# dome272/Paella

Measured on AMD Instinct MI355X. Metric: images/sec (whole node) + single-image ms, 256x256 @ 8 steps, higher is better.
Workload: dtype f32; 1 GPU; BASELINE configs[1]: Paella 573M-class (stand-in blocks=[4,8,4]) (570.3M params), 32x32 tokens = 256 px, 8 steps, CFG 8.0, CLIP-H-text only (S=4), batch 1 per GPU, + VQGAN f8 decode; denoiser=570m, sample_steps=8, noise=philox, submission=hip-graph replay, world_size_observed=1

## Files before the change

paella_amd/csrc/gemm.hip:

```cpp
#include "common.h"
#include "gemm_device.h"
#include "philox.h"
#include <stdio.h>
#include <stdlib.h>
#include "test_hooks.h"
#include <atomic>
#include <mutex>
#include <string>
#include <type_traits>
#include <utility>
#include <vector>

typedef unsigned int u32x4 __attribute__((ext_vector_type(4)));
typedef __bf16 bf16x8 __attribute__((ext_vector_type(8)));

template <typename F, int... Is>
__device__ __forceinline__ void static_for_impl(F& f, std::integer_sequence<int, Is...>) { (f(std::integral_constant<int, Is>{}), ...); }
template <int N, typename F>
__device__ __forceinline__ void static_for(F& f) { static_for_impl(f, std::make_integer_sequence<int, N>{}); }

struct SkPlan {
    int tiles_m, tiles_n;
    int KT;
    unsigned U;
    unsigned G;
    FastDiv dKT, dTM, dQ, dQ1;
    unsigned q, r;
    int stagger;
    int gm;
};

template <bool GROUPED>
__device__ __forceinline__ void sk_tile_coords(const SkPlan& p, int tile, int& tile_m, int& tile_n) {
    if (!GROUPED || p.gm >= p.tiles_m) {
        tile_n = (int)fast_div((unsigned)tile, p.dTM);
        tile_m = tile - tile_n * p.tiles_m;
    } else {
        const int width = p.gm * p.tiles_n;
        const int grp = tile / width, rem = tile - grp * width;
        const int first_m = grp * p.gm;
        const int gsz = min(p.tiles_m - first_m, p.gm);
        tile_n = rem / gsz;
        tile_m = first_m + (rem - tile_n * gsz);
    }
}

__device__ __forceinline__ unsigned sk_start(const SkPlan& p, unsigned g) { return g * p.q + min(g, p.r); }
__device__ __forceinline__ unsigned sk_owner(const SkPlan& p, unsigned x) {
    const unsigned big = p.r * (p.q + 1);
    return x < big ? fast_div(x, p.dQ1) : p.r + fast_div(x - big, p.dQ);
}

template <int AUX = 0>
__device__ __forceinline__ void dma_b128_to_lds(__amdgpu_buffer_rsrc_t rsrc, float* lds_wave_base, unsigned voffset, int soffset) {
#if defined(__HIP_DEVICE_COMPILE__)
    __builtin_amdgcn_raw_ptr_buffer_load_lds(rsrc, (__attribute__((address_space(3))) void*)lds_wave_base, 16, voffset, soffset, 0, AUX);
#endif
}
#ifndef PAELLA_RING_W_AUX
#define PAELLA_RING_W_AUX 2
#endif

__device__ __forceinline__ f32x4 mma_bf16(const f32x4 w, const f32x4 a, const f32x4 c) {
    return __builtin_amdgcn_mfma_f32_16x16x32_bf16(__builtin_bit_cast(bf16x8, w), __builtin_bit_cast(bf16x8, a), c, 0, 0, 0);
}

#ifdef PAELLA_GEMM_CLOCK_PROBE
__device__ unsigned long long g_clock_probe[2];
extern "C" int paella_probe_gemm_clock(unsigned long long* out2) {
    HIP_CHECK_RET(hipDeviceSynchronize());
    HIP_CHECK_RET(hipMemcpyFromSymbol(out2, HIP_SYMBOL(g_clock_probe), 2 * sizeof(unsigned long long)));
    return PAELLA_OK;
}
#endif

struct TileRes {
    int BM, BN;
    int tile_floats;
    int stage_floats;
    int flag_off;
    int tail_floats;
    int grn_scr;
    int lds_bytes;
    int side_samples;
};
constexpr TileRes tile_res(int WM, int WN, int TM, int TN, int APRO, bool TAIL, int BK, int RING) {
    const int BM = WM * TM * 16, BN = WN * TN * 16;
    const bool big = RING > 0 && WM * WN == 8;
    const int aux = RING == 0 ? 0 : (big && APRO == 1) ? 576 : APRO == 1 ? 512 : APRO == 4 ? 320 : 0;
    const int tile = (BM + BN) * BK, stage = tile + aux;
    const int flag_off = RING > 0 ? RING * stage : 2 * stage;
    const int tail = TAIL ? BM * WN * 2 : 0;
    const int scr = (RING > 0 && !big) ? WM * WN * TN * 16 : 0;
    return TileRes{BM, BN, tile, stage, flag_off, tail, scr, (flag_off + 16 + tail + scr) * 4, big ? 16 : 8};
}
constexpr int tile_wg_per_cu(int WM, int WN, int TM, int TN, int PD, int APRO, bool TAIL, int BK, bool DMA, int RING, bool BF) {
    const int NW = WM * WN, blocks = TM * TN;
    if (RING > 0) {
        const int wish = NW == 8 ? 1 : blocks == 1 ? (RING == 3 ? 5 : 4) : (blocks == 2 ? ((BF && APRO == 2 && TM == 2) ? 3 : 4) : 3);
        const int fit = (160 * 1024) / tile_res(WM, WN, TM, TN, APRO, TAIL, BK, RING).lds_bytes;
        return fit < wish ? (fit < 1 ? 1 : fit) : wish;
    }
    if (TAIL && DMA) return 4;
    if (TAIL && NW == 8 && blocks == 4) return 4;
    if (WM == 2 && WN == 2 && blocks == 1 && PD == 2 && BK == 32 && (APRO == 0 || APRO == 3)) return 5;
    if (DMA && NW == 4 && blocks == 16) return 2;
    if (NW == 8 && WM * TM == 8 && WN * TN == 4 && PD == 2 && BK == 32 && APRO == 0 && !TAIL) return 4;
    return 1;
}

template <int WM, int WN, int TM, int TN, int PD, int APRO, bool TAIL = false, int BK = 32, bool DMA = false, int RING = 0, bool BF = false, int EPI = EPI_RUNTIME, bool REQ = false>
__global__ __launch_bounds__(64 * WM * WN, tile_wg_per_cu(WM, WN, TM, TN, PD, APRO, TAIL, BK, DMA, RING, BF)) void gemm_nt_kernel(GemmArgs g, SkPlan p, float* __restrict__ slabs,
                                                               unsigned* __restrict__ tickets, unsigned slab_bytes) {
    constexpr TileRes RES = tile_res(WM, WN, TM, TN, APRO, TAIL, BK, RING);
    constexpr int BM = RES.BM, BN = RES.BN;
    constexpr int SL = BK / 4;
    constexpr int KG = BK / 16;
    constexpr int NW = WM * WN, NT = 64 * NW;
    constexpr int RP = NT / SL;
    constexpr int LA = (BM * SL + NT - 1) / NT, LB = (BN * SL + NT - 1) / NT;
    static_assert(NW == 4 || NW == 8, "4 or 8 waves per workgroup");
    static_assert(!REQ || TAIL, "the request form exists for the fused tail only");
    static_assert(PD == 1 || PD == 2, "prefetch ring depth 1 or 2");
    static_assert(BK == 32 || BK == 64, "K step of 32 or 64");
    static_assert(!BF || ((DMA || RING > 0) && (APRO == 0 || APRO == 2) && BK == 32), "bf16 operands: direct-to-LDS / ring variants, no operand transform");
    constexpr int ESZ = BF ? 2 : 4;
    constexpr bool DMA_W = DMA || RING > 0, DMA_A = (DMA && (APRO == 0 || APRO == 2)) || RING > 0;
    static_assert(!DMA || (PD == 1 && BK == 32 && (BM * SL) % NT == 0 && (BN * SL) % NT == 0), "DMA variant: 1-deep, K step 32, whole passes");
    constexpr bool PP = RING == 2;
    static_assert(!PP || (BF && NW == 8 && WM == 2 && WN == 4 && TM == 8 && TN == 4 && (APRO == 0 || APRO == 2)), "ping-pong tile: bf16 operands, 2 x 4 waves of 128x64 wave tiles");
    static_assert(RING == 0 || (RING >= 2 && RING <= 4 && !DMA && PD == 1 && BK == 32 && !TAIL && APRO != 3 && (NW == 4 || (TM == 4 && TN == 4 && RING == 3) || PP) && (BM * SL) % NT == 0 && (BN * SL) % NT == 0),
                  "ring variant: 3 or 4 LDS stages (2 for the ping-pong tile), 4 waves (or 8 waves of 64x64 / 128x64 wave tiles), K step 32, whole passes, no implicit convolution");
    static_assert(APRO != 4 || RING > 0, "the GRN-from-raw-statistics prologue exists on ring tiles only");
    constexpr bool BIG = RING > 0 && NW == 8;
    static_assert(!BIG || APRO != 4, "the 8-wave ring tile has no GRN-from-raw-statistics prologue");
    constexpr bool GRN_SIDE = RING > 0 && (APRO == 1 || APRO == 4);
    constexpr bool GRN_FIN = RING > 0 && !BIG;
    constexpr int TILE_FLOATS = RES.tile_floats, STAGE_FLOATS = RES.stage_floats, FLAG_OFF = RES.flag_off, TAIL_FLOATS = RES.tail_floats;
    static_assert(RES.side_samples == (BIG ? 16 : 8) && (RES.grn_scr > 0) == GRN_FIN, "tile_res() and the kernel agree on which ring tiles are BIG");
    __shared__ __attribute__((aligned(16))) float smem[RES.lds_bytes / 4];

    const unsigned G = p.G;
    unsigned gid = blockIdx.x;
    {
        const unsigned q = G >> 3, r = G & 7;
        const unsigned xcd = gid & 7, idx = gid >> 3;
        gid = xcd * q + min(xcd, r) + idx;
    }
    const unsigned u0 = sk_start(p, gid);
    const int n = (int)(p.q + (gid < p.r ? 1u : 0u));
    __builtin_assume(n > 0);
#ifdef PAELLA_GEMM_CLOCK_PROBE
    const unsigned long long cp_t0 = __builtin_readcyclecounter(), cp_w0 = wall_clock64();
#endif
    const int KT = p.KT;

    const int tid = threadIdx.x;
    const int lane_k = tid & 63;
    const int lane = lane_k;
    const int wave = __builtin_amdgcn_readfirstlane(tid >> 6);
    const int wm = wave / WN, wn = wave % WN;
    const int r16 = lane & 15, kq = lane >> 4;
    const int ldrow = tid / SL, ldc4 = tid % SL;

    f32x4 acc[TM][TN];
#pragma unroll
    for (int i = 0; i < TM; ++i)
#pragma unroll
        for (int j = 0; j < TN; ++j) acc[i][j] = f32x4{0.f, 0.f, 0.f, 0.f};

    struct Stage {
        f32x4 a[LA];
        f32x4 s[APRO == 1 ? LA : 1];
        f32x4 t;
        f32x4 b[LB];
        bool kok;
        bool ok[APRO == 3 ? LA : 1];
    };
    Stage R[PD];

    int ltile = (int)fast_div(u0, p.dKT);
    int lkt = (int)(u0 - (unsigned)ltile * (unsigned)KT);
    auto rsrc_of = [](const void* ptr, size_t bytes) {
        return __builtin_amdgcn_make_buffer_rsrc(const_cast<void*>(ptr), 0, (int)(bytes > 0xffffffffull ? 0xffffffffull : bytes), 0x00020000);
    };
    const char* const Abase = BF ? reinterpret_cast<const char*>(g.A16) : reinterpret_cast<const char*>(g.A);
    const char* const Wbase = BF ? reinterpret_cast<const char*>(g.W16) : reinterpret_cast<const char*>(g.W);
    const size_t a_bytes = APRO == 3 ? (size_t)(g.M / (g.cv.Ho * g.cv.Wo)) * g.cv.Hi * g.cv.Wi * g.cv.C * sizeof(float)
                                     : ((size_t)(g.M - 1) * g.lda + g.K) * ESZ;
    const size_t w_bytes = ((size_t)(g.N - 1) * g.ldw + g.K) * ESZ;
    __amdgpu_buffer_rsrc_t rsrcA = rsrc_of(Abase, a_bytes), rsrcW = rsrc_of(Wbase, w_bytes);
    __amdgpu_buffer_rsrc_t rsrcS = rsrc_of(g.A, 16);
    const __amdgpu_buffer_rsrc_t rsrcT = rsrc_of((APRO == 1 || APRO == 4) ? g.a_shift : g.A, (APRO == 1 || APRO == 4) ? (size_t)g.K * sizeof(float) : 16);
    const __amdgpu_buffer_rsrc_t rsrcG = rsrc_of(APRO == 4 ? g.grn_gamma : g.A, APRO == 4 ? (size_t)g.K * sizeof(float) : 16);
    unsigned aoff[LA], soff[APRO == 1 ? LA : 1], boff[LB];
    unsigned aux_s_off2 = 0;
    unsigned aux_s_off = 0;
    int cy[APRO == 3 ? LA : 1], cx[APRO == 3 ? LA : 1];
    int ltap = 0, lc0 = 0;
    auto set_tile = [&](int tile) __attribute__((always_inline)) {
        int tile_m, tile_n;
        sk_tile_coords<(BM >= 64)>(p, tile, tile_m, tile_n);
        const int m0 = tile_m * BM, n0 = tile_n * BN;
        size_t a_base;
        int img0 = 0, smp0 = 0;
        if (APRO == 3) {
            img0 = m0 / (g.cv.Ho * g.cv.Wo);
            a_base = (size_t)img0 * g.cv.Hi * g.cv.Wi * g.cv.C * sizeof(float);
        } else {
            a_base = (size_t)m0 * g.lda * ESZ;
        }
        rsrcA = rsrc_of(Abase + a_base, a_bytes - a_base);
        const size_t w_base = (size_t)n0 * g.ldw * ESZ;
        rsrcW = rsrc_of(Wbase + w_base, w_bytes - w_base);
        if (APRO == 1 || APRO == 4) {
            smp0 = (int)fast_div((unsigned)m0, g.a_rps_div);
            const size_t s_bytes = (size_t)(fast_div((unsigned)(g.M - 1), g.a_rps_div) + 1) * g.K * sizeof(float), s_base = (size_t)smp0 * g.K * sizeof(float);
            rsrcS = rsrc_of((APRO == 4 ? g.grn_gx : g.a_scale) + (size_t)smp0 * g.K, s_bytes - s_base);
        }
#pragma unroll
        for (int i = 0; i < LA; ++i) {
            const int gmc = min(m0 + ldrow + i * RP, g.M - 1);
            if (APRO == 3) {
                const int hw = g.cv.Ho * g.cv.Wo;
                const int bimg = gmc / hw, rem = gmc - bimg * hw;
                const int yo = rem / g.cv.Wo, xo = rem - yo * g.cv.Wo;
                cy[i] = yo * g.cv.stride;
                cx[i] = xo * g.cv.stride;
                aoff[i] = (unsigned)(bimg - img0) * (unsigned)(g.cv.Hi * g.cv.Wi);
            } else {
                aoff[i] = (unsigned)(gmc - m0) * (unsigned)g.lda * (unsigned)ESZ + (unsigned)((DMA_A ? (ldc4 ^ (ldrow & (SL - 1))) : ldc4) * 16);
            }
            if (APRO == 1 && RING == 0) soff[i] = ((unsigned)((int)fast_div((unsigned)gmc, g.a_rps_div) - smp0) * (unsigned)g.K + (unsigned)(ldc4 * 4)) * 4u;
        }
        if (GRN_SIDE) {
            const int last = (int)fast_div((unsigned)(g.M - 1), g.a_rps_div) - smp0;
            aux_s_off = ((unsigned)min(lane_k >> 3, last) * (unsigned)g.K + (unsigned)((lane_k & 7) * 4)) * 4u;
            if (BIG) aux_s_off2 = ((unsigned)min(8 + (lane_k >> 3), last) * (unsigned)g.K + (unsigned)((lane_k & 7) * 4)) * 4u;
        }
#pragma unroll
        for (int i = 0; i < LB; ++i) boff[i] = (unsigned)(min(n0 + ldrow + i * RP, g.N - 1) - n0) * (unsigned)g.ldw * (unsigned)ESZ + (unsigned)((DMA_W ? (ldc4 ^ (ldrow & (SL - 1))) : ldc4) * 16);
    };
    set_tile(ltile);
    if (APRO == 3) {
        ltap = (lkt * BK) / g.cv.C;
        lc0 = lkt * BK - ltap * g.cv.C;
    }
    float fr_mu[APRO == 2 ? TM : 1], fr_rs[APRO == 2 ? TM : 1];
    float fr_mu_lo[APRO == 2 ? TM : 1];
    bool ln_dir[APRO == 2 ? TM : 1];
    constexpr bool BF_FIX = BF && APRO == 2 && NW == 4;
    bool ln_any = false;
    int ln_row0 = 0;
    const int ln_tile0 = ltile;
    auto ln_row_stats = [&]() __attribute__((always_inline)) {
        if constexpr (APRO == 2) {
            int ln_tm, ln_tn;
            sk_tile_coords<(BM >= 64)>(p, ln_tile0, ln_tm, ln_tn);
            ln_row0 = ln_tm * BM;
            int lane_l = (NW == 8 && BF) ? (int)__builtin_amdgcn_mbcnt_hi(~0u, __builtin_amdgcn_mbcnt_lo(~0u, 0u)) : lane_k;
            asm volatile("" : "+v"(lane_l));
            const int r16 = lane_l & 15;
            if (PP || g.ln_row) {
#pragma unroll
                for (int i = 0; i < TM; ++i) {
                    const int gmc = min(ln_tm * BM + (wm * TM + i) * 16 + r16, g.M - 1);
                    const f32x4 v = *reinterpret_cast<const f32x4*>(g.ln_row + (size_t)gmc * 4);
                    fr_mu[i] = v[0]; fr_rs[i] = v[1]; fr_mu_lo[i] = v[2];
                    if constexpr (BF) {
                        ln_dir[i] = false;
                        const bool pre = g.A != nullptr && v[3] > g.ln_fold_ratio;
                        if (pre) { fr_mu[i] = 0.f; fr_rs[i] = 1.f; }
                        if (g.ln_guard_count) ln_any = ln_any || __builtin_amdgcn_ballot_w64(pre) != 0;
                    } else {
                        ln_dir[i] = __builtin_amdgcn_ballot_w64(v[3] > g.ln_fold_ratio) != 0;
                        ln_any = ln_any || ln_dir[i];
                    }
                }
                if (g.ln_guard_count && ln_any && lane_l == 0) atomicAdd(g.ln_guard_count, 1u);
                return;
            }
            const int nch = g.ln_nblk >> 1;
#pragma unroll
            for (int i = 0; i < TM; ++i) {
                const int gmc = min(ln_tm * BM + (wm * TM + i) * 16 + r16, g.M - 1);
                const float* st0 = g.ln_stats + (size_t)gmc * g.ln_nblk * 2;
                const bool vec = (((size_t)gmc * g.ln_nblk) & 1) == 0;
                RowStatAcc acc;
                if (vec) {
                    const f32x4* stp = reinterpret_cast<const f32x4*>(st0);
                    int j = kq;
                    for (; j + 12 < nch; j += 16) {
                        const f32x4 v0 = stp[j], v1 = stp[j + 4], v2 = stp[j + 8], v3 = stp[j + 12];
                        acc.add(v0[0], v0[1]); acc.add(v0[2], v0[3]); acc.add(v1[0], v1[1]); acc.add(v1[2], v1[3]);
                        acc.add(v2[0], v2[1]); acc.add(v2[2], v2[3]); acc.add(v3[0], v3[1]); acc.add(v3[2], v3[3]);
                    }
                    for (; j < nch; j += 4) {
                        const f32x4 v0 = stp[j];
                        acc.add(v0[0], v0[1]); acc.add(v0[2], v0[3]);
                    }
                    if ((g.ln_nblk & 1) && kq == 0) acc.add(st0[2 * (g.ln_nblk - 1)], st0[2 * (g.ln_nblk - 1) + 1]);
                } else {
                    for (int j = kq; j < g.ln_nblk; j += 4) acc.add(st0[2 * j], st0[2 * j + 1]);
                }
                acc.S += __shfl_xor(acc.S, 16, 64); acc.Q += __shfl_xor(acc.Q, 16, 64); acc.M += __shfl_xor(acc.M, 16, 64);
                acc.S += __shfl_xor(acc.S, 32, 64); acc.Q += __shfl_xor(acc.Q, 32, 64); acc.M += __shfl_xor(acc.M, 32, 64);
                acc.finish(g.K, g.ln_eps, fr_mu[i], fr_rs[i]);
                fr_mu_lo[i] = (float)(acc.S / (double)g.K - (double)fr_mu[i]);
                ln_dir[i] = (!BF || (BF_FIX && g.A != nullptr)) && __builtin_amdgcn_ballot_w64(fabsf(fr_mu[i]) * fr_rs[i] > g.ln_fold_ratio) != 0;
                ln_any = ln_any || ln_dir[i];
            }
            if (g.ln_guard_count && ln_any && lane_k == 0) atomicAdd(g.ln_guard_count, 1u);
        }
    };
    auto ln_fix = [&](f32x4& a, int i, int kbase) __attribute__((always_inline)) {
        if constexpr (APRO == 2 && !BF) {
            if (ln_dir[i]) {
#pragma unroll
                for (int e = 0; e < 4; ++e) a[e] = (kbase + e < g.K) ? ((a[e] - fr_mu[i]) - fr_mu_lo[i]) * fr_rs[i] : 0.f;
            }
        }
        if constexpr (BF_FIX) {
            if (ln_dir[i]) {
                const int gm = min(ln_row0 + (wm * TM + i) * 16 + r16, g.M - 1);
                const float* src = g.A + (size_t)gm * g.lda + 2 * kbase;
                typedef __bf16 bf16x4_t __attribute__((ext_vector_type(4)));
                f32x4 v = *reinterpret_cast<const f32x4*>(src);
#pragma unroll
                for (int e = 0; e < 4; ++e) v[e] = ((v[e] - fr_mu[i]) - fr_mu_lo[i]) * fr_rs[i];
                const bf16x4_t lo = __builtin_convertvector(v, bf16x4_t);
                v = *reinterpret_cast<const f32x4*>(src + 4);
#pragma unroll
                for (int e = 0; e < 4; ++e) v[e] = ((v[e] - fr_mu[i]) - fr_mu_lo[i]) * fr_rs[i];
                const bf16x4_t hi = __builtin_convertvector(v, bf16x4_t);
                a = __builtin_bit_cast(f32x4, __builtin_shufflevector(lo, hi, 0, 1, 2, 3, 4, 5, 6, 7));
            }
        }
    };
    int kt_cur = 0;

    auto load_unit = [&](Stage& r, int dma_slot) __attribute__((always_inline)) {
        float* dAs = smem + dma_slot * (RING > 0 ? STAGE_FLOATS : TILE_FLOATS) + (wave * (64 / SL)) * BK;
        float* dBs = dAs + BM * BK;
        const int kofs = lkt * (BK * 4);
        if constexpr (RING > 0) {
#pragma unroll
            for (int i = 0; i < LA; ++i) dma_b128_to_lds(rsrcA, dAs + i * RP * BK, aoff[i], kofs);
#pragma unroll
            for (int i = 0; i < LB; ++i) dma_b128_to_lds<((BIG || TM * TN != 1) ? 0 : PAELLA_RING_W_AUX)>(rsrcW, dBs + i * RP * BK, boff[i], kofs);
            if (GRN_SIDE && wave == NW - 1) {
                float* dX = smem + dma_slot * STAGE_FLOATS + TILE_FLOATS;
                if (BIG) {
                    if (lane_k < 8) dma_b128_to_lds(rsrcT, dX, (unsigned)(lane_k * 16), kofs);
                    dma_b128_to_lds(rsrcS, dX + 64, aux_s_off, kofs);
                    dma_b128_to_lds(rsrcS, dX + 64 + 256, aux_s_off2, kofs);
                } else if (APRO == 4) {
                    if (lane_k < 8) {
                        dma_b128_to_lds(rsrcT, dX, (unsigned)(lane_k * 16), kofs);
                        dma_b128_to_lds(rsrcG, dX + 32, (unsigned)(lane_k * 16), kofs);
                    }
                    dma_b128_to_lds(rsrcS, dX + 64, aux_s_off, kofs);
                } else {
                    dma_b128_to_lds(rsrcT, dX, (unsigned)((lane_k & 7) * 16), kofs);
                    dma_b128_to_lds(rsrcS, dX + 256, aux_s_off, kofs);
                }
            }
            return;
        }
        int oy = 0, ox = 0;
        if (APRO == 3) {
            oy = g.cv.oy0 + g.cv.tsign * (ltap >> g.cv.tw_log2);
            ox = g.cv.ox0 + g.cv.tsign * (ltap & ((1 << g.cv.tw_log2) - 1));
        }
#pragma unroll
        for (int i = 0; i < LA; ++i) {
            if (APRO == 3) {
                const int yy = cy[i] + oy, xx = cx[i] + ox;
                r.ok[i] = (unsigned)yy < (unsigned)g.cv.Hi && (unsigned)xx < (unsigned)g.cv.Wi;
                const unsigned pos = aoff[i] + (unsigned)(min(max(yy, 0), g.cv.Hi - 1) * g.cv.Wi + min(max(xx, 0), g.cv.Wi - 1));
                r.a[i] = __builtin_bit_cast(f32x4, __builtin_amdgcn_raw_buffer_load_b128(rsrcA, (pos * (unsigned)g.cv.C + (unsigned)(ldc4 * 4)) * 4u, lc0 * 4, 0));
            } else if (DMA_A) {
                dma_b128_to_lds(rsrcA, dAs + i * RP * BK, aoff[i], kofs);
            } else {
                r.a[i] = __builtin_bit_cast(f32x4, __builtin_amdgcn_raw_buffer_load_b128(rsrcA, aoff[i], kofs, 0));
            }
            if (APRO == 1) r.s[i] = __builtin_bit_cast(f32x4, __builtin_amdgcn_raw_buffer_load_b128(rsrcS, soff[i], kofs, 0));
        }
        if (APRO == 1) r.t = __builtin_bit_cast(f32x4, __builtin_amdgcn_raw_buffer_load_b128(rsrcT, (unsigned)(ldc4 * 16), kofs, 0));
#pragma unroll
        for (int i = 0; i < LB; ++i) {
            if (DMA_W) dma_b128_to_lds(rsrcW, dBs + i * RP * BK, boff[i], kofs);
            else r.b[i] = __builtin_bit_cast(f32x4, __builtin_amdgcn_raw_buffer_load_b128(rsrcW, boff[i], kofs, 0));
        }
        r.kok = lkt * BK + ldc4 * 4 < g.K;
    };
    auto store_unit = [&](const Stage& r, int slot) __attribute__((always_inline)) {
        float* As = smem + slot * TILE_FLOATS;
        float* Bs = As + BM * BK;
#pragma unroll
        for (int i = 0; i < (DMA_A ? 0 : LA); ++i) {
            const int row = ldrow + i * RP;
            f32x4 v = r.a[i];
            if (APRO == 1) v = v * r.s[i] + r.t;
            if (!r.kok || (APRO == 3 && !r.ok[i])) v = f32x4{0.f, 0.f, 0.f, 0.f};
            if (LA * RP == BM || row < BM) *reinterpret_cast<f32x4*>(As + row * BK + ((ldc4 ^ (row & (SL - 1))) << 2)) = v;
        }
#pragma unroll
        for (int i = 0; i < (DMA_W ? 0 : LB); ++i) {
            const int row = ldrow + i * RP;
            if (LB * RP == BN || row < BN) *reinterpret_cast<f32x4*>(Bs + row * BK + ((ldc4 ^ (row & (SL - 1))) << 2)) = r.b[i];
        }
        if (DMA) asm volatile("s_waitcnt vmcnt(0)" ::: "memory");
    };
    constexpr bool PIPE = (NW == 8 && PD == 1 && TM * TN == 8 && BK == 32 && !TAIL);
    f32x4 Fa[KG][TM], Fb[KG][TN];
    auto read_group = [&](auto kk_tag, int slot, int kt) __attribute__((always_inline)) {
        constexpr int kk = decltype(kk_tag)::value;
        const float* As = smem + slot * TILE_FLOATS;
        const float* Bs = As + BM * BK;
        const int c4 = kk * 4 + kq;
#pragma unroll
        for (int i = 0; i < TM; ++i) {
            const int row = (wm * TM + i) * 16 + r16;
            Fa[kk][i] = *reinterpret_cast<const f32x4*>(As + row * BK + ((c4 ^ (row & (SL - 1))) << 2));
        }
        if (APRO == 2 && ln_any) {
#pragma unroll
            for (int i = 0; i < TM; ++i) ln_fix(Fa[kk][i], i, kt * BK + c4 * 4);
        }
#pragma unroll
        for (int j = 0; j < TN; ++j) {
            const int row = (wn * TN + j) * 16 + r16;
            Fb[kk][j] = *reinterpret_cast<const f32x4*>(Bs + row * BK + ((c4 ^ (row & (SL - 1))) << 2));
        }
    };
    auto mfma_group = [&](auto kk_tag, auto e0_tag, auto e1_tag) __attribute__((always_inline)) {
        constexpr int kk = decltype(kk_tag)::value, e0 = decltype(e0_tag)::value, e1 = decltype(e1_tag)::value;
        if constexpr (BF) {
#pragma unroll
            for (int ij = e0 * TM * TN / 4; ij < e1 * TM * TN / 4; ++ij) acc[ij / TN][ij % TN] = mma_bf16(Fb[kk][ij % TN], Fa[kk][ij / TN], acc[ij / TN][ij % TN]);
        } else {
#pragma unroll
            for (int e = e0; e < e1; ++e)
#pragma unroll
                for (int i = 0; i < TM; ++i)
#pragma unroll
                    for (int j = 0; j < TN; ++j)
                        acc[i][j] = __builtin_amdgcn_mfma_f32_16x16x4f32(Fb[kk][j][e], Fa[kk][i][e], acc[i][j], 0, 0, 0);
        }
    };
    constexpr bool DUAL = (TM * TN == 1);
    f32x4 acc2 = f32x4{0.f, 0.f, 0.f, 0.f};
    auto compute = [&](int slot) __attribute__((always_inline)) {
        const float* As = smem + slot * TILE_FLOATS;
        const float* Bs = As + BM * BK;
        constexpr bool FRAG_FIRST = (TM * TN <= 2) || (NW == 8 && TM + TN <= 6 && PD == 1);
        if constexpr (FRAG_FIRST) {
            f32x4 af[KG][TM], bf[KG][TN];
#pragma unroll
            for (int kk = 0; kk < KG; ++kk) {
                const int c4 = kk * 4 + kq;
#pragma unroll
                for (int i = 0; i < TM; ++i) {
                    const int row = (wm * TM + i) * 16 + r16;
                    af[kk][i] = *reinterpret_cast<const f32x4*>(As + row * BK + ((c4 ^ (row & (SL - 1))) << 2));
                }
#pragma unroll
                for (int j = 0; j < TN; ++j) {
                    const int row = (wn * TN + j) * 16 + r16;
                    bf[kk][j] = *reinterpret_cast<const f32x4*>(Bs + row * BK + ((c4 ^ (row & (SL - 1))) << 2));
                }
            }
            if (APRO == 2 && ln_any) {
#pragma unroll
                for (int kk = 0; kk < KG; ++kk)
#pragma unroll
                    for (int i = 0; i < TM; ++i) ln_fix(af[kk][i], i, kt_cur * BK + (kk * 4 + kq) * 4);
            }
            if constexpr (BF) {
                if (DUAL) {
#pragma unroll
                    for (int kk = 0; kk < KG; kk += 2) {
                        acc[0][0] = mma_bf16(bf[kk][0], af[kk][0], acc[0][0]);
                        acc2 = mma_bf16(bf[kk + 1][0], af[kk + 1][0], acc2);
                    }
                } else {
#pragma unroll
                    for (int kk = 0; kk < KG; ++kk)
#pragma unroll
                        for (int i = 0; i < TM; ++i)
#pragma unroll
                            for (int j = 0; j < TN; ++j) acc[i][j] = mma_bf16(bf[kk][j], af[kk][i], acc[i][j]);
                }
            } else if (DUAL) {
#pragma unroll
                for (int kk = 0; kk < KG; kk += 2)
#pragma unroll
                    for (int e = 0; e < 4; ++e) {
                        acc[0][0] = __builtin_amdgcn_mfma_f32_16x16x4f32(bf[kk][0][e], af[kk][0][e], acc[0][0], 0, 0, 0);
                        acc2 = __builtin_amdgcn_mfma_f32_16x16x4f32(bf[kk + 1][0][e], af[kk + 1][0][e], acc2, 0, 0, 0);
                    }
            } else {
#pragma unroll
                for (int kk = 0; kk < KG; ++kk)
#pragma unroll
                    for (int e = 0; e < 4; ++e)
#pragma unroll
                        for (int i = 0; i < TM; ++i)
#pragma unroll
                            for (int j = 0; j < TN; ++j)
                                acc[i][j] = __builtin_amdgcn_mfma_f32_16x16x4f32(bf[kk][j][e], af[kk][i][e], acc[i][j], 0, 0, 0);
            }
        } else {
#pragma unroll
            for (int kk = 0; kk < KG; ++kk) {
                f32x4 af[TM], bf[TN];
                const int c4 = kk * 4 + kq;
#pragma unroll
                for (int i = 0; i < TM; ++i) {
                    const int row = (wm * TM + i) * 16 + r16;
                    af[i] = *reinterpret_cast<const f32x4*>(As + row * BK + ((c4 ^ (row & (SL - 1))) << 2));
                }
#pragma unroll
                for (int j = 0; j < TN; ++j) {
                    const int row = (wn * TN + j) * 16 + r16;
                    bf[j] = *reinterpret_cast<const f32x4*>(Bs + row * BK + ((c4 ^ (row & (SL - 1))) << 2));
                }
                if (APRO == 2 && ln_any) {
#pragma unroll
                    for (int i = 0; i < TM; ++i) ln_fix(af[i], i, kt_cur * BK + c4 * 4);
                }
                if constexpr (BF) {
#pragma unroll
                    for (int i = 0; i < TM; ++i)
#pragma unroll
                        for (int j = 0; j < TN; ++j) acc[i][j] = mma_bf16(bf[j], af[i], acc[i][j]);
                } else {
#pragma unroll
                    for (int e = 0; e < 4; ++e)
#pragma unroll
                        for (int i = 0; i < TM; ++i)
#pragma unroll
                            for (int j = 0; j < TN; ++j)
                                acc[i][j] = __builtin_amdgcn_mfma_f32_16x16x4f32(bf[j][e], af[i][e], acc[i][j], 0, 0, 0);
                }
            }
        }
    };

    constexpr bool TAIL_AHEAD = TAIL && DMA;
    float tlq[TAIL_AHEAD ? TM * TN : 1][4];
    int tlq_tile = -1;
    int tail_cur_tile = -1;
    auto tail_req_row = [&](int m, uint64_t& rseed, int64_t& ctr_row, uint64_t& rstep) __attribute__((always_inline)) {
        const int mc = min(m, g.M - 1);
        const unsigned b = fast_div((unsigned)mc, g.rq.rps_div);
        rseed = g.rq.seeds[b];
        ctr_row = mc - (int)b * g.rq.rows_per_sample;
        if (g.rq.step) rstep = (uint64_t)g.rq.step[b];
        return b;
    };
    auto tail_draw = [&](int tile) __attribute__((always_inline)) {
        if constexpr (TAIL_AHEAD) {
            if (g.ft.mode != 1) {
                const FusedTail& ft = g.ft;
                int tile_m, tile_n;
                sk_tile_coords<(BM >= 64)>(p, tile, tile_m, tile_n);
                const uint64_t seed = ft.seed + (ft.seed_ptr ? *ft.seed_ptr : 0ull);
                const int64_t row_off = ft.row_offset + (ft.row_offset_ptr ? *ft.row_offset_ptr : 0);
                const int L4 = g.N >> 2;
#pragma unroll
                for (int i = 0; i < TM; ++i) {
                    const int m = tile_m * BM + (wm * TM + i) * 16 + r16;
                    uint64_t rseed = seed;
                    int64_t ctr_row = m + row_off;
                    uint64_t rstep = ft.offset;
                    if constexpr (REQ) tail_req_row(m, rseed, ctr_row, rstep);
#pragma unroll
                    for (int j = 0; j < TN; ++j) {
                        const int nn = tile_n * BN + (wn * TN + j) * 16 + kq * 4;
                        uint32_t rb[4];
                        philox4x32(rseed, (uint64_t)ctr_row * L4 + (nn >> 2), rstep, rb);
#pragma unroll
                        for (int e = 0; e < 4; ++e) tlq[i * TN + j][e] = log_exp1(rb[e]);
                    }
// ... 184 lines not shown
        sk_tile_coords<(BM >= 64)>(p, tile, tile_m, tile_n);
        int lane = PP ? (int)__builtin_amdgcn_mbcnt_hi(~0u, __builtin_amdgcn_mbcnt_lo(~0u, 0u)) : lane_k;
        asm volatile("" : "+v"(lane));
        const int r16 = lane & 15, kq = lane >> 4;
        if (DUAL) { acc[0][0] += acc2; acc2 = f32x4{0.f, 0.f, 0.f, 0.f}; }
        bool finish = true;
        if (!(k0 == 0 && k1 == KT)) {
            const unsigned mybase = (2u * gid + (first ? 0u : 1u)) * SLOT_BYTES + (unsigned)(wave * FR * 4);
#pragma unroll
            for (int i = 0; i < TM; ++i)
#pragma unroll
                for (int j = 0; j < TN; ++j)
                    __builtin_amdgcn_raw_buffer_store_b128(__builtin_bit_cast(u32x4, acc[i][j]), rsrc,
                                                           mybase + ((i * TN + j) * 64 + lane) * 16, 0, 16);
            asm volatile("s_waitcnt vmcnt(0)" ::: "memory");
            __syncthreads();
            unsigned* sflag = reinterpret_cast<unsigned*>(smem + FLAG_OFF);
            if (tid == 0) sflag[0] = __hip_atomic_fetch_add(tickets + tile, 1u, __ATOMIC_RELAXED, __HIP_MEMORY_SCOPE_AGENT);
            __syncthreads();
            const unsigned tb = (unsigned)tile * (unsigned)KT;
            const unsigned g_first = sk_owner(p, tb);
            const unsigned g_last = sk_owner(p, tb + (unsigned)KT - 1u);
            finish = sflag[0] == g_last - g_first;
            if (finish) {
                if (tid == 0) __hip_atomic_store(tickets + tile, 0u, __ATOMIC_RELAXED, __HIP_MEMORY_SCOPE_AGENT);
                const unsigned off_first = (2u * g_first + (sk_start(p, g_first) < tb ? 1u : 0u)) * SLOT_BYTES;
                const unsigned wbase = (unsigned)(wave * FR * 4);
#pragma unroll
                for (int i = 0; i < TM; ++i)
#pragma unroll
                    for (int j = 0; j < TN; ++j) {
                        const unsigned fo = wbase + ((i * TN + j) * 64 + lane) * 16;
                        f32x4 v = __builtin_bit_cast(f32x4, __builtin_amdgcn_raw_buffer_load_b128(rsrc, off_first + fo, 0, 16));
                        unsigned gp = g_first + 1;
                        for (; gp + 3 <= g_last; gp += 4) {
                            const f32x4 a0 = __builtin_bit_cast(f32x4, __builtin_amdgcn_raw_buffer_load_b128(rsrc, (2u * gp + 0u) * SLOT_BYTES + fo, 0, 16));
                            const f32x4 a1 = __builtin_bit_cast(f32x4, __builtin_amdgcn_raw_buffer_load_b128(rsrc, (2u * gp + 2u) * SLOT_BYTES + fo, 0, 16));
                            const f32x4 a2 = __builtin_bit_cast(f32x4, __builtin_amdgcn_raw_buffer_load_b128(rsrc, (2u * gp + 4u) * SLOT_BYTES + fo, 0, 16));
                            const f32x4 a3 = __builtin_bit_cast(f32x4, __builtin_amdgcn_raw_buffer_load_b128(rsrc, (2u * gp + 6u) * SLOT_BYTES + fo, 0, 16));
                            v += a0; v += a1; v += a2; v += a3;
                        }
                        for (; gp <= g_last; ++gp)
                            v += __builtin_bit_cast(f32x4, __builtin_amdgcn_raw_buffer_load_b128(rsrc, 2u * gp * SLOT_BYTES + fo, 0, 16));
                        acc[i][j] = v;
                    }
            }
        }
        tail_cur_tile = tile;
        if (finish) epilogue(tile_m * BM, tile_n * BN, r16, kq);
#pragma unroll
        for (int i = 0; i < TM; ++i)
#pragma unroll
            for (int j = 0; j < TN; ++j) acc[i][j] = f32x4{0.f, 0.f, 0.f, 0.f};
    };

    int loaded = 0;
    if constexpr (RING > 0) {
        int sidx[GRN_SIDE ? TM : 1];
        float rinv[(APRO == 4) ? TM : 1];
        int rinv_tile_m = -1;
        auto enter_tile = [&](int tile) __attribute__((always_inline)) {
            if (!GRN_SIDE) return;
            int tile_m, tile_n;
            sk_tile_coords<(BM >= 64)>(p, tile, tile_m, tile_n);
            const int m0 = tile_m * BM, smp0 = (int)fast_div((unsigned)m0, g.a_rps_div);
#pragma unroll
            for (int i = 0; i < TM; ++i) sidx[i] = (int)fast_div((unsigned)min(m0 + (wm * TM + i) * 16 + r16, g.M - 1), g.a_rps_div) - smp0;
            if (APRO == 4 && tile_m != rinv_tile_m) {
                rinv_tile_m = tile_m;
#pragma unroll
                for (int i = 0; i < TM; ++i) {
                    const int smp = __builtin_amdgcn_readfirstlane(smp0 + sidx[i]);
                    const float* sp = g.grn_part + (size_t)smp * g.grn_np;
                    float sm = 0.f;
                    for (int j = lane_k; j < g.grn_np; j += 64) sm += sp[j];
#pragma unroll
                    for (int o = 32; o > 0; o >>= 1) sm += __shfl_xor(sm, o, 64);
                    rinv[i] = 1.0f / (sm / (float)g.K + 1e-6f);
                }
            }
        };
        auto compute_ring = [&](int cs, int kt_ring) __attribute__((always_inline)) {
            const float* As = smem + cs * STAGE_FLOATS;
            const float* Bs = As + BM * BK;
            f32x4 af[KG][TM], bf[KG][TN];
#pragma unroll
            for (int kk = 0; kk < KG; ++kk) {
                const int c4 = kk * 4 + kq;
#pragma unroll
                for (int i = 0; i < TM; ++i) {
                    const int row = (wm * TM + i) * 16 + r16;
                    af[kk][i] = *reinterpret_cast<const f32x4*>(As + row * BK + ((c4 ^ (row & (SL - 1))) << 2));
                }
#pragma unroll
                for (int j = 0; j < TN; ++j) {
                    const int row = (wn * TN + j) * 16 + r16;
                    bf[kk][j] = *reinterpret_cast<const f32x4*>(Bs + row * BK + ((c4 ^ (row & (SL - 1))) << 2));
                }
            }
            if (APRO == 2 && ln_any) {
#pragma unroll
                for (int kk = 0; kk < KG; ++kk)
#pragma unroll
                    for (int i = 0; i < TM; ++i) ln_fix(af[kk][i], i, BF_FIX ? kt_ring * BK + (kk * 4 + kq) * 4 : 0);
            }
            if (APRO == 1) {
                const float* X = Bs + BN * BK;
#pragma unroll
                for (int kk = 0; kk < KG; ++kk) {
                    const int c4 = kk * 4 + kq;
                    const f32x4 t = *reinterpret_cast<const f32x4*>(X + c4 * 4);
#pragma unroll
                    for (int i = 0; i < TM; ++i) {
                        const f32x4 sc = *reinterpret_cast<const f32x4*>(X + 256 + sidx[i] * 32 + c4 * 4);
                        af[kk][i] = af[kk][i] * sc + t;
                    }
                }
            }
            if (APRO == 4) {
                const float* X = Bs + BN * BK;
#pragma unroll
                for (int kk = 0; kk < KG; ++kk) {
                    const int c4 = kk * 4 + kq;
                    const f32x4 t = *reinterpret_cast<const f32x4*>(X + c4 * 4);
                    const f32x4 gm = *reinterpret_cast<const f32x4*>(X + 32 + c4 * 4);
#pragma unroll
                    for (int i = 0; i < TM; ++i) {
                        const f32x4 gx = *reinterpret_cast<const f32x4*>(X + 64 + sidx[i] * 32 + c4 * 4);
                        const f32x4 sc = gm * gx * rinv[i] + 1.0f;
                        af[kk][i] = af[kk][i] * sc + t;
                    }
                }
            }
            if constexpr (BF) {
                if (TM * TN == 1) {
#pragma unroll
                    for (int kk = 0; kk < KG; kk += 2) {
                        acc[0][0] = mma_bf16(bf[kk][0], af[kk][0], acc[0][0]);
                        acc2 = mma_bf16(bf[kk + 1][0], af[kk + 1][0], acc2);
                    }
                } else {
#pragma unroll
                    for (int kk = 0; kk < KG; ++kk)
#pragma unroll
                        for (int i = 0; i < TM; ++i)
#pragma unroll
                            for (int j = 0; j < TN; ++j) acc[i][j] = mma_bf16(bf[kk][j], af[kk][i], acc[i][j]);
                }
            } else if (TM * TN == 1) {
#pragma unroll
                for (int kk = 0; kk < KG; kk += 2)
#pragma unroll
                    for (int e = 0; e < 4; ++e) {
                        acc[0][0] = __builtin_amdgcn_mfma_f32_16x16x4f32(bf[kk][0][e], af[kk][0][e], acc[0][0], 0, 0, 0);
                        acc2 = __builtin_amdgcn_mfma_f32_16x16x4f32(bf[kk + 1][0][e], af[kk + 1][0][e], acc2, 0, 0, 0);
                    }
            } else {
#pragma unroll
                for (int kk = 0; kk < KG; ++kk)
#pragma unroll
                    for (int e = 0; e < 4; ++e)
#pragma unroll
                        for (int i = 0; i < TM; ++i)
#pragma unroll
                            for (int j = 0; j < TN; ++j)
                                acc[i][j] = __builtin_amdgcn_mfma_f32_16x16x4f32(bf[kk][j][e], af[kk][i][e], acc[i][j], 0, 0, 0);
            }
        };
        auto fetch_ring = [&](int stage) __attribute__((always_inline)) {
            load_unit(R[0], stage);
            if (++loaded < n) {
                if (++lkt == KT) {
                    lkt = 0;
                    ++ltile;
                    set_tile(ltile);
                }
            }
        };
        constexpr int PER_UNIT = LA + LB;
        constexpr int SIDE_DMAS = (APRO == 4 || BIG) ? 3 : 2;
        if constexpr (PP) {
            using I0 = std::integral_constant<int, 0>;
            using I1 = std::integral_constant<int, 1>;
            using I2 = std::integral_constant<int, 2>;
            using I3 = std::integral_constant<int, 3>;
            using I4 = std::integral_constant<int, 4>;
            int lbuf = 0;
            auto pp_issue = [&](auto sec_tag) __attribute__((always_inline)) {
                constexpr int sec = decltype(sec_tag)::value;
                float* dAs = smem + lbuf * STAGE_FLOATS + (wave * (64 / SL)) * BK;
                float* dBs = dAs + BM * BK;
                const int kofs = lkt * (BK * 4);
                if constexpr (sec == 0) {
                    dma_b128_to_lds(rsrcA, dAs, aoff[0], kofs);
                    dma_b128_to_lds(rsrcA, dAs + 2 * RP * BK, aoff[2], kofs);
                } else if constexpr (sec == 1) {
                    dma_b128_to_lds(rsrcW, dBs, boff[0], kofs);
                    dma_b128_to_lds(rsrcW, dBs + RP * BK, boff[1], kofs);
                } else if constexpr (sec == 2) {
                    dma_b128_to_lds(rsrcW, dBs + 2 * RP * BK, boff[2], kofs);
                    dma_b128_to_lds(rsrcW, dBs + 3 * RP * BK, boff[3], kofs);
                } else {
                    dma_b128_to_lds(rsrcA, dAs + RP * BK, aoff[1], kofs);
                    dma_b128_to_lds(rsrcA, dAs + 3 * RP * BK, aoff[3], kofs);
                    lbuf ^= 1;
                    if (++loaded < n) {
                        if (++lkt == KT) {
                            lkt = 0;
                            ++ltile;
                            set_tile(ltile);
                        }
                    }
                }
            };
            f32x4 PA[2][4], PBl[2][2], PBh[2][2];
            auto rdA = [&](int st, auto ib_tag) __attribute__((always_inline)) {
                constexpr int ib = decltype(ib_tag)::value;
                const float* As = smem + st * STAGE_FLOATS;
#pragma unroll
                for (int kk = 0; kk < 2; ++kk) {
                    const int c4 = kk * 4 + kq;
#pragma unroll
                    for (int i = 0; i < 4; ++i) {
                        const int row = (wm * TM + ib + i) * 16 + r16;
                        PA[kk][i] = *reinterpret_cast<const f32x4*>(As + row * BK + ((c4 ^ (row & (SL - 1))) << 2));
                    }
                }
            };
            auto rdB = [&](f32x4 (&dst)[2][2], int st, auto jb_tag) __attribute__((always_inline)) {
                constexpr int jb = decltype(jb_tag)::value;
                const float* Bs = smem + st * STAGE_FLOATS + BM * BK;
#pragma unroll
                for (int kk = 0; kk < 2; ++kk) {
                    const int c4 = kk * 4 + kq;
#pragma unroll
                    for (int j = 0; j < 2; ++j) {
                        const int row = (wn * TN + jb + j) * 16 + r16;
                        dst[kk][j] = *reinterpret_cast<const f32x4*>(Bs + row * BK + ((c4 ^ (row & (SL - 1))) << 2));
                    }
                }
            };
            auto mm = [&](auto ib_tag, auto jb_tag, const f32x4 (&pb)[2][2]) __attribute__((always_inline)) {
                constexpr int ib = decltype(ib_tag)::value, jb = decltype(jb_tag)::value;
                __builtin_amdgcn_sched_barrier(0);
                __builtin_amdgcn_s_barrier();
                asm volatile("s_waitcnt lgkmcnt(0)" ::: "memory");
                __builtin_amdgcn_sched_barrier(0);
                __builtin_amdgcn_s_setprio(1);
#pragma unroll
                for (int kk = 0; kk < 2; ++kk)
#pragma unroll
                    for (int i = 0; i < 4; ++i)
#pragma unroll
                        for (int j = 0; j < 2; ++j) acc[ib + i][jb + j] = mma_bf16(pb[kk][j], PA[kk][i], acc[ib + i][jb + j]);
                __builtin_amdgcn_s_setprio(0);
                __builtin_amdgcn_sched_barrier(0);
                __builtin_amdgcn_s_barrier();
                asm volatile("" ::: "memory");
            };
            pp_issue(I0{}); pp_issue(I1{}); pp_issue(I2{}); pp_issue(I3{}); pp_issue(I0{}); pp_issue(I1{});
            asm volatile("s_waitcnt vmcnt(6)" ::: "memory");
            __builtin_amdgcn_s_barrier();
            asm volatile("" ::: "memory");
            int cbuf = 0;
            int ctile = (int)fast_div(u0, p.dKT);
            int ckt = (int)(u0 - (unsigned)ctile * (unsigned)KT);
            bool first_seg = true;
            for (int i = 0; i < n;) {
                const int seg_len = min(KT - ckt, n - i);
                if (wm == 1) __builtin_amdgcn_s_barrier();
                asm volatile("" ::: "memory");
                for (int s2 = 0; s2 < seg_len; ++s2) {
                    rdA(cbuf, I0{});
                    rdB(PBl, cbuf, I0{});
                    __builtin_amdgcn_sched_barrier(0);
                    pp_issue(I2{});
                    mm(I0{}, I0{}, PBl);
                    rdB(PBh, cbuf, I2{});
                    __builtin_amdgcn_sched_barrier(0);
                    pp_issue(I3{});
                    asm volatile("s_waitcnt vmcnt(8)" ::: "memory");
                    mm(I0{}, I2{}, PBh);
                    rdA(cbuf, I4{});
                    __builtin_amdgcn_sched_barrier(0);
                    pp_issue(I0{});
                    mm(I4{}, I2{}, PBh);
                    pp_issue(I1{});
                    asm volatile("s_waitcnt vmcnt(6)" ::: "memory");
                    mm(I4{}, I0{}, PBl);
                    cbuf ^= 1;
                }
                if (wm == 0) __builtin_amdgcn_s_barrier();
                asm volatile("" ::: "memory");
                if (i + seg_len == n) asm volatile("s_waitcnt vmcnt(0)" ::: "memory");
                if (first_seg) ln_row_stats();
                flush(ctile, ckt, ckt + seg_len, first_seg);
                first_seg = false;
                i += seg_len;
                ckt += seg_len;
                if (ckt == KT) { ckt = 0; ++ctile; }
            }
            return;
        }
#pragma unroll
        for (int j = 0; j < RING - 1; ++j) fetch_ring(j);
        if constexpr (!BIG) ln_row_stats();
        int cs = 0, ls = RING - 1;
        int ctile = (int)fast_div(u0, p.dKT);
        int ckt = (int)(u0 - (unsigned)ctile * (unsigned)KT);
        bool first_seg = true;
        if constexpr (BIG && !PP) {
            f32x4 Sg[APRO == 1 ? KG : 1][APRO == 1 ? TM : 1], Tg[APRO == 1 ? KG : 1];
            auto big_read = [&](auto kk_tag, int st) __attribute__((always_inline)) {
                constexpr int kk = decltype(kk_tag)::value;
                const float* As = smem + st * STAGE_FLOATS;
                const float* Bs = As + BM * BK;
                const int c4 = kk * 4 + kq;
#pragma unroll
                for (int i = 0; i < TM; ++i) {
                    const int row = (wm * TM + i) * 16 + r16;
                    Fa[kk][i] = *reinterpret_cast<const f32x4*>(As + row * BK + ((c4 ^ (row & (SL - 1))) << 2));
                }
#pragma unroll
                for (int j = 0; j < TN; ++j) {
                    const int row = (wn * TN + j) * 16 + r16;
                    Fb[kk][j] = *reinterpret_cast<const f32x4*>(Bs + row * BK + ((c4 ^ (row & (SL - 1))) << 2));
                }
                if constexpr (APRO == 1) {
                    const float* X = Bs + BN * BK;
                    Tg[kk] = *reinterpret_cast<const f32x4*>(X + c4 * 4);
#pragma unroll
                    for (int i = 0; i < TM; ++i) Sg[kk][i] = *reinterpret_cast<const f32x4*>(X + 64 + sidx[i] * 32 + c4 * 4);
                }
            };
            auto big_xform = [&](auto kk_tag, int kt_ring) __attribute__((always_inline)) {
                constexpr int kk = decltype(kk_tag)::value;
                if constexpr (APRO == 1) {
#pragma unroll
                    for (int i = 0; i < TM; ++i) Fa[kk][i] = Fa[kk][i] * Sg[kk][i] + Tg[kk];
                }
                if (APRO == 2 && ln_any) {
#pragma unroll
                    for (int i = 0; i < TM; ++i) ln_fix(Fa[kk][i], i, 0);
                }
            };
            using I0 = std::integral_constant<int, 0>;
            using I1 = std::integral_constant<int, 1>;
            using I4 = std::integral_constant<int, 4>;
            static_assert(KG == 2, "two k groups per K step");
            const bool late = p.stagger == 1 ? wave >= NW / 2 : (p.stagger == 2 ? (wave & 1) != 0 : false);
            for (int i = 0; i < n;) {
                const int seg_len = min(KT - ckt, n - i);
                enter_tile(ctile);
                bool pend = false;
                for (int s2 = 0; s2 < seg_len; ++s2) {
                    if (GRN_SIDE && wave == NW - 1) asm volatile("s_waitcnt vmcnt(%0) lgkmcnt(0)" ::"n"((RING - 2) * (PER_UNIT + SIDE_DMAS)) : "memory");
                    else asm volatile("s_waitcnt vmcnt(%0) lgkmcnt(0)" ::"n"((RING - 2) * PER_UNIT) : "memory");
                    __builtin_amdgcn_s_barrier();
                    asm volatile("" ::: "memory");
                    if (!late) {
                        fetch_ring(ls);
                        __builtin_amdgcn_sched_barrier(0);
                        big_read(I0{}, cs);
                    }
                    __builtin_amdgcn_sched_barrier(0);
                    if (pend) {
                        big_xform(I1{}, ckt + s2 - 1);
                        mfma_group(I1{}, I0{}, I4{});
                    }
                    __builtin_amdgcn_sched_barrier(0);
                    if (late) {
                        fetch_ring(ls);
                        __builtin_amdgcn_sched_barrier(0);
                        big_read(I0{}, cs);
                    }
                    __builtin_amdgcn_sched_barrier(0);
                    big_read(I1{}, cs);
                    __builtin_amdgcn_sched_barrier(0);
                    big_xform(I0{}, ckt + s2);
                    mfma_group(I0{}, I0{}, I4{});
                    __builtin_amdgcn_sched_barrier(0);
                    pend = true;
                    cs = cs + 1 == RING ? 0 : cs + 1;
                    ls = ls + 1 == RING ? 0 : ls + 1;
                }
                big_xform(I1{}, ckt + seg_len - 1);
                mfma_group(I1{}, I0{}, I4{});
                __builtin_amdgcn_sched_barrier(0);
                if (i + seg_len == n) asm volatile("s_waitcnt vmcnt(0)" ::: "memory");
                if (first_seg) ln_row_stats();
                flush(ctile, ckt, ckt + seg_len, first_seg);
                first_seg = false;
                i += seg_len;
                ckt += seg_len;
                if (ckt == KT) { ckt = 0; ++ctile; }
            }
            return;
        }
        for (int i = 0; i < n;) {
            const int seg_len = min(KT - ckt, n - i);
            enter_tile(ctile);
            for (int s2 = 0; s2 < seg_len; ++s2) {
                if (GRN_SIDE && wave == NW - 1) asm volatile("s_waitcnt vmcnt(%0)" ::"n"((RING - 2) * (PER_UNIT + SIDE_DMAS)) : "memory");
                else asm volatile("s_waitcnt vmcnt(%0)" ::"n"((RING - 2) * PER_UNIT) : "memory");
                __builtin_amdgcn_s_barrier();
                asm volatile("" ::: "memory");
                fetch_ring(ls);
                __builtin_amdgcn_sched_barrier(0);
                compute_ring(cs, ckt + s2);
                __builtin_amdgcn_sched_barrier(0);
                cs = cs + 1 == RING ? 0 : cs + 1;
                ls = ls + 1 == RING ? 0 : ls + 1;
            }
            if (i + seg_len == n) asm volatile("s_waitcnt vmcnt(0)" ::: "memory");
            flush(ctile, ckt, ckt + seg_len, first_seg);
            first_seg = false;
            i += seg_len;
            ckt += seg_len;
            if (ckt == KT) { ckt = 0; ++ctile; }
        }
        return;
    }
    auto fetch = [&](Stage& r, int dma_slot) __attribute__((always_inline)) {
        load_unit(r, dma_slot);
        if (++loaded < n) {
            if (APRO == 3 && (lc0 += BK) == g.cv.C) { lc0 = 0; ++ltap; }
            if (++lkt == KT) {
                lkt = 0;
                ltap = 0;
                lc0 = 0;
                ++ltile;
                set_tile(ltile);
            }
        }
    };
    const int tile_first = (int)fast_div(u0, p.dKT);
#pragma unroll
    for (int j = 0; j < PD; ++j) fetch(R[j], 0);
    ln_row_stats();
    if constexpr (TAIL_AHEAD) tail_draw(tile_first);
    store_unit(R[0], 0);
    __syncthreads();
    if constexpr (PIPE) read_group(std::integral_constant<int, 0>{}, 0, (int)(u0 - fast_div(u0, p.dKT) * (unsigned)KT));

    int ctile = (int)fast_div(u0, p.dKT);
    int ckt = (int)(u0 - (unsigned)ctile * (unsigned)KT);
    bool first_seg = true;
    int slot = 0;
    auto step = [&](Stage& rf, const Stage& rs, auto sl_tag) __attribute__((always_inline)) {
        constexpr int sl = decltype(sl_tag)::value;
        using I0 = std::integral_constant<int, 0>;
        using I1 = std::integral_constant<int, 1>;
        using I2 = std::integral_constant<int, 2>;
        using I4 = std::integral_constant<int, 4>;
        fetch(rf, sl ^ 1);
        __builtin_amdgcn_sched_barrier(0);
        if constexpr (PIPE) {
            read_group(I1{}, sl, kt_cur);
            __builtin_amdgcn_sched_barrier(0);
            mfma_group(I0{}, I0{}, I4{});
            mfma_group(I1{}, I0{}, I2{});
            __builtin_amdgcn_sched_barrier(0);
            store_unit(rs, sl ^ 1);
            __syncthreads();
            read_group(I0{}, sl ^ 1, kt_cur + 1);
            __builtin_amdgcn_sched_barrier(0);
            mfma_group(I1{}, I2{}, I4{});
            __builtin_amdgcn_sched_barrier(0);
        } else {
            compute(sl);
            __builtin_amdgcn_sched_barrier(0);
            store_unit(rs, sl ^ 1);
            __syncthreads();
        }
        ++kt_cur;
    };
    auto run_segment = [&](auto s0_tag, int len) __attribute__((always_inline)) {
        constexpr int S0 = decltype(s0_tag)::value;
        int s = 0;
        if constexpr (PD == 1) {
            for (; s + 2 <= len; s += 2) {
                step(R[0], R[0], std::integral_constant<int, S0>{});
                step(R[0], R[0], std::integral_constant<int, S0 ^ 1>{});
            }
            if (s < len) step(R[0], R[0], std::integral_constant<int, S0>{});
        } else {
            for (; s + 2 <= len; s += 2) {
                step(R[0], R[1], std::integral_constant<int, S0>{});
                step(R[1], R[0], std::integral_constant<int, S0 ^ 1>{});
            }
            if (s < len) {
                step(R[0], R[1], std::integral_constant<int, S0>{});
                R[1] = R[0];
            }
        }
    };
    for (int i = 0; i < n;) {
        const int seg_len = min(KT - ckt, n - i);
        kt_cur = ckt;
        if (slot == 0) run_segment(std::integral_constant<int, 0>{}, seg_len);
        else run_segment(std::integral_constant<int, 1>{}, seg_len);
        slot ^= seg_len & 1;
        flush(ctile, ckt, ckt + seg_len, first_seg);
        first_seg = false;
        i += seg_len;
        ckt += seg_len;
        if (ckt == KT) { ckt = 0; ++ctile; }
    }
#ifdef PAELLA_GEMM_CLOCK_PROBE
    if (gid == (G >> 1) && tid == 0) {
        g_clock_probe[0] = __builtin_readcyclecounter() - cp_t0;
        g_clock_probe[1] = wall_clock64() - cp_w0;
    }
#endif
}

enum : unsigned {
    V_F32 = 1,
    V_CONV = 2,
    V_DMA = 4,
    V_DMA_PLAIN = 8,
    V_RING = 16,
    V_BF16 = 32,
    V_TAIL = 64,
};
struct Tile {
    int wm, wn, tm, tn;
    int pd, bk, ring;
    unsigned var;
    constexpr bool has(unsigned v) const { return (var & v) == v; }
    constexpr int waves() const { return wm * wn; }
    constexpr TileRes res(int apro = 0) const { return tile_res(wm, wn, tm, tn, apro, false, bk, ring); }
};
static constexpr Tile kCfgs[] = {
    {2, 2, 4, 4, 1, 32, 0, V_F32 | V_DMA | V_DMA_PLAIN},
    {2, 2, 4, 2, 2, 32, 0, V_F32},
    {2, 2, 2, 2, 2, 32, 0, V_F32 | V_CONV | V_TAIL},
    {2, 2, 2, 1, 2, 32, 0, V_F32},
    {2, 2, 1, 2, 2, 32, 0, V_F32},
    {2, 2, 1, 1, 2, 32, 0, V_F32 | V_CONV},
    {1, 4, 1, 1, 2, 32, 0, V_F32},
    {1, 4, 1, 2, 2, 32, 0, V_F32},
    {1, 4, 2, 2, 2, 32, 0, V_F32},
    {4, 2, 2, 4, 1, 32, 0, V_F32 | V_CONV | V_TAIL},
    {2, 4, 4, 2, 1, 32, 0, V_F32 | V_CONV | V_DMA | V_BF16},
    {4, 1, 2, 2, 2, 32, 0, V_F32},
    {4, 1, 2, 4, 2, 32, 0, V_F32},
    {4, 1, 1, 4, 2, 32, 0, V_F32},
    {4, 2, 2, 2, 2, 32, 0, V_F32 | V_CONV | V_TAIL},
    {8, 1, 2, 2, 2, 32, 0, V_F32},
    {8, 1, 2, 4, 1, 32, 0, V_F32},
    {8, 1, 1, 4, 2, 32, 0, V_F32},
    {2, 2, 2, 2, 1, 32, 0, V_F32 | V_CONV | V_DMA | V_BF16 | V_TAIL},
    {2, 2, 1, 1, 1, 32, 0, V_F32 | V_CONV | V_DMA | V_BF16},
    {4, 1, 2, 4, 1, 32, 0, V_F32},
    {4, 1, 1, 2, 2, 32, 0, V_F32},
    {2, 2, 1, 4, 2, 32, 0, V_F32},
    {1, 4, 2, 1, 2, 32, 0, V_F32},
    {2, 2, 1, 1, 2, 64, 0, V_F32},
    {2, 2, 1, 1, 1, 64, 0, V_F32},
    {2, 2, 2, 2, 1, 64, 0, V_F32},
    {4, 1, 2, 2, 1, 64, 0, V_F32},
    {2, 2, 1, 2, 1, 64, 0, V_F32},
    {4, 2, 2, 2, 1, 64, 0, V_F32},
    {2, 2, 1, 1, 1, 32, 3, V_RING | V_BF16},
    {2, 2, 1, 1, 1, 32, 4, V_RING | V_BF16},
    {2, 2, 1, 2, 1, 32, 3, V_RING | V_BF16},
    {2, 2, 2, 1, 1, 32, 3, V_RING | V_BF16},
    {2, 2, 2, 2, 1, 32, 3, V_RING | V_BF16},
    {2, 2, 1, 2, 1, 32, 4, V_RING | V_BF16},
    {4, 2, 4, 4, 1, 32, 3, V_BF16},
    {2, 4, 8, 4, 1, 32, 2, V_BF16},
};
static constexpr int kNumCfgs = sizeof(kCfgs) / sizeof(kCfgs[0]);
using TileIds = std::make_integer_sequence<int, kNumCfgs>;
int gemm_num_tile_configs() { return kNumCfgs; }
static bool cfg_has(int cfg, unsigned v) { return cfg >= 0 && cfg < kNumCfgs && kCfgs[cfg].has(v); }
static std::string ids_with(unsigned v) {
    std::string s;
    for (int i = 0; i < kNumCfgs; ++i) {
        if (!kCfgs[i].has(v)) continue;
        int j = i;
        while (cfg_has(j + 1, v)) ++j;
        s += (s.empty() ? "" : ", ") + std::to_string(i);
        if (j > i) s += (j > i + 1 ? ".." : ", ") + std::to_string(j);
        i = j;
    }
    return s;
}

static std::atomic<int> g_gemm_raster_gm{8};
extern "C" int paella_test_gemm_raster(int gm) { g_gemm_raster_gm = gm; return PAELLA_OK; }
static std::atomic<int> g_gemm_dma{1};
extern "C" int paella_test_gemm_dma(int on) { g_gemm_dma = on != 0; return PAELLA_OK; }

static int epi_class(const GemmArgs& g, bool stores = true) {
    const Epilogue& e = g.ep;
    if (e.alpha != 1.0f || (stores && (e.store_mode != STORE_PLAIN || e.remap_in > 0 || e.c16 || !g.C))) return EPI_RUNTIME;
    return (e.bias ? EPI_BIAS : 0) | (e.act == ACT_GELU ? EPI_GELU : 0) | (e.residual ? EPI_RESID : 0) | (e.ts ? EPI_TS : 0) |
           (e.rowstat_out ? EPI_ROWSTAT : 0) | (e.sumsq_out ? EPI_SUMSQ : 0) | (e.grn_gx_out ? EPI_GRNFIN : 0);
}
static std::atomic<int> g_gemm_epi_spec{1};
extern "C" int paella_test_gemm_epi_specialise(int on) { g_gemm_epi_spec = on != 0; return PAELLA_OK; }
static thread_local int g_last_epi = EPI_RUNTIME;
static thread_local int g_last_cfg = -1;
static thread_local long long g_last_G = 0, g_last_T = 0, g_last_bf = 0;
// ... 632 lines not shown
```

Measured before the change: 45.66 images/sec.

## Prefetch LayerNorm row stats ahead of ring fetch and split reduction across warps

Result: faster. 46.18 images/sec (median of 6 runs) (+1.1%).

```diff
diff --git a/paella_amd/csrc/gemm.hip b/paella_amd/csrc/gemm.hip
--- a/paella_amd/csrc/gemm.hip
+++ b/paella_amd/csrc/gemm.hip
@@ -253,6 +253,25 @@
     bool ln_any = false;
     int ln_row0 = 0;
     const int ln_tile0 = ltile;
+    constexpr bool LN_AHEAD = APRO == 2 && RING > 0 && NW == 4 && WN == 2 && !BF;
+    constexpr int LN_NP = TM == 1 ? 5 : 2;
+    f32x4 ln_pre[LN_AHEAD ? TM : 1][LN_AHEAD ? LN_NP : 1];
+    auto ln_issue = [&]() __attribute__((always_inline)) {
+        if constexpr (LN_AHEAD) {
+            if (!g.ln_row) {
+                int ln_tm, ln_tn;
+                sk_tile_coords<(BM >= 64)>(p, ln_tile0, ln_tm, ln_tn);
+                const int nch = g.ln_nblk >> 1;
+#pragma unroll
+                for (int i = 0; i < TM; ++i) {
+                    const int gmc = min(ln_tm * BM + (wm * TM + i) * 16 + r16, g.M - 1);
+                    const f32x4* stp = reinterpret_cast<const f32x4*>(g.ln_stats + (size_t)gmc * g.ln_nblk * 2);
+#pragma unroll
+                    for (int c = 0; c < LN_NP; ++c) ln_pre[i][c] = stp[min(kq + 4 * wn + 8 * c, nch - 1)];
+                }
+            }
+        }
+    };
     auto ln_row_stats = [&]() __attribute__((always_inline)) {
         if constexpr (APRO == 2) {
             int ln_tm, ln_tn;
@@ -281,6 +300,50 @@
                 return;
             }
             const int nch = g.ln_nblk >> 1;
+            if constexpr (LN_AHEAD) {
+                RowStatAcc part[TM];
+                double* const xch = reinterpret_cast<double*>(smem + (RING - 1) * STAGE_FLOATS);
+#pragma unroll
+                for (int i = 0; i < TM; ++i) {
+                    RowStatAcc acc;
+#pragma unroll
+                    for (int c = 0; c < LN_NP; ++c) {
+                        const bool in = kq + 4 * wn + 8 * c < nch;
+                        const f32x4 v = ln_pre[i][c];
+                        acc.add(in ? v[0] : 0.f, in ? v[1] : 0.f); acc.add(in ? v[2] : 0.f, in ? v[3] : 0.f);
+                    }
+                    if (kq + 4 * wn + 8 * LN_NP < nch) {
+                        const int gmc = min(ln_tm * BM + (wm * TM + i) * 16 + r16, g.M - 1);
+                        const f32x4* stp = reinterpret_cast<const f32x4*>(g.ln_stats + (size_t)gmc * g.ln_nblk * 2);
+                        for (int j = kq + 4 * wn + 8 * LN_NP; j < nch; j += 8) {
+                            const f32x4 v = stp[j];
+                            acc.add(v[0], v[1]); acc.add(v[2], v[3]);
+                        }
+                    }
+                    acc.S += __shfl_xor(acc.S, 16, 64); acc.Q += __shfl_xor(acc.Q, 16, 64); acc.M += __shfl_xor(acc.M, 16, 64);
+                    acc.S += __shfl_xor(acc.S, 32, 64); acc.Q += __shfl_xor(acc.Q, 32, 64); acc.M += __shfl_xor(acc.M, 32, 64);
+                    if (kq == 0) {
+                        double* dst = xch + (wn * BM + (wm * TM + i) * 16 + r16) * 3;
+                        dst[0] = acc.S; dst[1] = acc.Q; dst[2] = acc.M;
+                    }
+                    part[i] = acc;
+                }
+                asm volatile("s_waitcnt lgkmcnt(0)" ::: "memory");
+                __builtin_amdgcn_s_barrier();
+                asm volatile("" ::: "memory");
+#pragma unroll
+                for (int i = 0; i < TM; ++i) {
+                    const double* src = xch + ((wn ^ 1) * BM + (wm * TM + i) * 16 + r16) * 3;
+                    RowStatAcc acc = part[i];
+                    acc.S += src[0]; acc.Q += src[1]; acc.M += src[2];
+                    acc.finish(g.K, g.ln_eps, fr_mu[i], fr_rs[i]);
+                    fr_mu_lo[i] = (float)(acc.S / (double)g.K - (double)fr_mu[i]);
+                    ln_dir[i] = __builtin_amdgcn_ballot_w64(fabsf(fr_mu[i]) * fr_rs[i] > g.ln_fold_ratio) != 0;
+                    ln_any = ln_any || ln_dir[i];
+                }
+                if (g.ln_guard_count && ln_any && lane_k == 0) atomicAdd(g.ln_guard_count, 1u);
+                return;
+            }
 #pragma unroll
             for (int i = 0; i < TM; ++i) {
                 const int gmc = min(ln_tm * BM + (wm * TM + i) * 16 + r16, g.M - 1);
@@ -1071,6 +1134,7 @@
             }
             return;
         }
+        ln_issue();
 #pragma unroll
         for (int j = 0; j < RING - 1; ++j) fetch_ring(j);
         if constexpr (!BIG) ln_row_stats();
```
